# luigifcruz/radio-core

Hardware: AMD Instinct MI355X
Metric: IQ Msamples/s through Tuner+WBFM at 1024 channels (higher is better)
Workload: dtype f32

## Files before the change

### include/rcfm_tools.h

```cpp
#ifndef RCFM_TOOLS_H
#define RCFM_TOOLS_H

#include "rcfm.h"

#ifdef __cplusplus
extern "C" {
#endif

typedef struct rcfm_arena_s* rcfm_arena_t;

int rcfm_arena_create(size_t block_bytes, rcfm_arena_t* out);
int rcfm_arena_adopt(void* base, size_t bytes, rcfm_arena_t* out);
int rcfm_arena_bind(rcfm_arena_t arena);
int rcfm_arena_stats(rcfm_arena_t arena, size_t* reserved_bytes, size_t* used_bytes, size_t* live_pieces);
int rcfm_arena_destroy(rcfm_arena_t arena);


enum { RCFM_TUNER_OPT_NARROW_TILES = 1,
       RCFM_TUNER_OPT_ALIGNED_PLAN = 2 };
int rcfm_tuner_set_option(rcfm_tuner_t t, int option, int value);

enum { RCFM_OPT_LDS_CHAIN = 1, RCFM_OPT_FUSED_TILES = 2, RCFM_OPT_PHASE_LINK = 3, RCFM_OPT_PILOT_CHAIN = 6, RCFM_OPT_DECIM_TILE = 7,
       RCFM_OPT_LDS_DEEMPH = 8, RCFM_OPT_PILOT_BLOCKED = 9 };
int rcfm_demod_get_option(rcfm_demod_t d, int option, int* value);


typedef struct rcfm_fft_pass {
    int32_t L, nstages, radix[8];
    int64_t n_o1, n_o2, n_inner;
    int64_t in_o1, in_o2, in_i, in_l;
    int64_t out_o1, out_o2, out_i, out_k;
    int64_t tw_o1, tw_o2, tw_i;
    int32_t has_twiddle, load_along_l;
    int64_t in_t, out_t;
    int32_t flat_outer;
    int32_t reserved_;
} rcfm_fft_pass;
typedef struct rcfm_fft_plan {
// ... 23 lines not shown
```

### radio-core_amd/csrc/api_internal.h

```cpp
#pragma once

#include <algorithm>
#include <atomic>
#include <cstdlib>
#include <map>
#include <memory>
#include <mutex>
#include <string>
#include <vector>

#include "common.h"
#include "fft_engine.h"
#include "fft_plan.h"
#include "fused_passes.h"
#include "kernels.h"
#include "lds_chain.h"

#define TILE_CALL(narrow_tiles, fn, ...) ((narrow_tiles) ? ::rcfm::narrow::fn(__VA_ARGS__) : ::rcfm::fn(__VA_ARGS__))

namespace rcfm {

constexpr double kPi = 3.14159265358979323846;


// ... 1 lines not shown
    int64_t n = 0, m = 0;
    int nmin = 0, nyq = 0, nneg = 0;
    int nyq_mode = NYQ_NONE;
    float w_merge = 0.f;
    float nyq_factor = 1.f;
    float scale = 1.f;
    DeviceBuffer wpos, wneg;
    DeviceBuffer wr;

    void build(int64_t n_, int64_t m_, double a0, bool complex_input);
};

std::vector<double> firwin_bandpass(int numtaps, double lo, double hi);
std::vector<float> zero_phase_kernel(const float* b, int nb);
void deemphasis_design(int64_t fs, double tau, float* taps51, float* zi50);

struct PlanCache {
    std::map<int, std::unique_ptr<FftPlan>> by_batch;
    FftPlan& get(FftKind kind, size_t n, int batch, bool in_place, size_t& work_need) {
        auto it = by_batch.find(batch);
        if (it == by_batch.end())
            it = by_batch.emplace(batch, std::make_unique<FftPlan>(kind, n, (size_t)batch, in_place)).first;
        work_need = std::max(work_need, it->second->work_bytes());
        return *it->second;
    }
};

enum Stage : int {
    ST_TUNER_FFT = 0,
    ST_TUNER_GATHER,
// ... 174 lines not shown
```

### radio-core_amd/csrc/demod.hip

```cpp

#include <cmath>
#include <cstring>

#include "api_internal.h"

using namespace rcfm;

struct rcfm_demod_s {
    Arena* arena = arena_enter_handle();
    ~rcfm_demod_s() {
        drop_graphs();
        if (cap_stream) (void)hipStreamDestroy(cap_stream);
        arena_leave_handle(arena);
    }
    int kind = 0, C = 0, B = 0, A = 0, ch = 1, chunk = 1;
    double tau = 75e-6;
    float taps_h[51];
    float zi_h[50];
    float pilot_h[41];
    float pilot_g_h[41];
    DeviceBuffer taps, pilot_g;
    struct StateBuf : DeviceBuffer {
        hipEvent_t ev = nullptr;
        bool armed = false, recorded = false;
// ... 16 lines not shown
    float* state_ptr() const { return state_buf->as<float>() + state_off; }
    float* state_at(int first) const { return state_ptr() + (size_t)first * ch * 50; }
    float side_tap = 0.23f;
    ResampleGeom geom;
    PlanCache r2c_B, c2c_inv_B, c2c_fwd_B, c2c_inv_A, c2r_A;
    std::unique_ptr<FftEngine> eng_B, eng_A;
    std::unique_ptr<FftEngine> eng_Ad;
    std::unique_ptr<FftEngine> eng_Bi;
    DeviceBuffer buf_Ti;
    bool opt_lds_chain = true;
    bool opt_pilot_chain = true;
    bool opt_decim_tile = true;
    bool opt_pilot_blocked = true;
    bool opt_phase_link = true;
    bool opt_lds_deemph = true;
    int opt_narrow = kNarrowDefault;
    bool opt_graph = false;
    struct GraphSlot {
        const void* iq;
        void* audio;
        const float* state;
        int first;
        hipGraphExec_t exec;
        uint64_t used;
    };
    std::vector<GraphSlot> graphs;
    GraphSlot last_call{nullptr, nullptr, nullptr, -1, nullptr, 0};
    hipStream_t cap_stream = nullptr;
    uint64_t graph_tick = 0;
    void drop_graphs() {
// ... 92 lines not shown
    int audio_pitch() const {
        if (!eng_Ad || kind != RCFM_WBFM || !deemph_fused()) return 0;
        const int64_t n1 = eng_Ad->row_length();
        return (n1 % 16 == 0 || (n1 * 2) % 4 != 0) ? 0 : (int)((n1 + 15) / 16 * 16);
    }

    bool deemph_geometric() const {
        if (!(taps_h[0] == 0.f && taps_h[1] > 0.f)) return false;
        for (int i = 1; i < 50; ++i)
            if (std::fabs((double)taps_h[i + 1] * taps_h[1] - (double)taps_h[i] * taps_h[2]) >
                4e-7 * (double)taps_h[i] * taps_h[1] + 1e-36)
                return false;
        return true;
    }

    DeviceBuffer taps_sfx;
    const float* taps_sfx_dev() {
        if (taps_sfx.bytes() == 0) {
            float h[102];
            for (int i = 0; i < 51; ++i) h[i] = taps_h[i];
            double acc = 0.0;
            for (int i = 50; i >= 0; --i) {
                h[51 + i] = (float)acc;
                acc += (double)taps_h[i];
            }
            taps_sfx.upload(h, sizeof(h));
        }
        return taps_sfx.as<float>();
    }

// ... 100 lines not shown
            }
            paired = true;
        } else {
            {
                StageTimer tm(ST_FFT_REAL_B, s);
                TILE_CALL(nw, fused_real_pair_fft, *eng_B, p, U2, T, cnt, packed ? kKeepLowerHalf : -1, s);
            }
            if (eng_Bi && opt_pilot_chain) {
                StageTimer tm(ST_IFFT_B, s);
                paired = !packed ? TILE_CALL(nw, fused_hilbert_pair_ifft_mix_fft, *eng_Bi, *eng_B, U2, m, buf_Ti.as<float2>(), T, cnt, s)
                                 : TILE_CALL(nw, fused_hilbert_packed_ifft_mix_fft, *eng_Bi, *eng_B, U2, p, m,
                                             buf_Ti.as<float2>(), T, cnt, s);
            }
        }
        if (paired && eng_Ad && opt_decim_tile && TILE_CALL(nw, fused_fft_decim_ifft_applies, *eng_B, *eng_Ad, cnt)) {
            const int pitch = audio_pitch();
            {
                StageTimer tm(ST_FFT_B, s);
                TILE_CALL(nw, fused_fft_decim_ifft, *eng_B, *eng_Ad, T, V, TA, cnt, geom.wr.as<float>(), geom.scale,
                          buf_dc.as<float2>(), s, pitch);
            }
            run_deemph(reinterpret_cast<float*>(V), audio, first, cnt, s, false, pitch ? (int)eng_Ad->row_length() : 0, pitch);
            return;
        }
        if (paired) {
            StageTimer tm(ST_FFT_B, s);
            TILE_CALL(nw, fused_fft_last_pruned, *eng_B, T, Z, cnt, std::min(A, B) / 2, s);
        } else {
            {
                StageTimer tm(ST_IFFT_B, s);
// ... 291 lines not shown
    });
}

int rcfm_demod_set_option(rcfm_demod_t d, int option, int value) {
    return guarded([&] {
        RC_REQUIRE(d, RCFM_ERR_ARG, "NULL handle");
        d->drop_graphs();
        switch (option) {
            case RCFM_OPT_GRAPH: d->opt_graph = value != 0; break;
            case RCFM_OPT_LDS_CHAIN: d->opt_lds_chain = value != 0; break;
            case RCFM_OPT_FUSED_TILES: d->opt_pilot_chain = d->opt_decim_tile = value != 0; break;
            case RCFM_OPT_PILOT_CHAIN: d->opt_pilot_chain = value != 0; break;
            case RCFM_OPT_DECIM_TILE: d->opt_decim_tile = value != 0; break;
            case RCFM_OPT_PILOT_BLOCKED: d->opt_pilot_blocked = value != 0; break;
            case RCFM_OPT_LDS_DEEMPH: d->opt_lds_deemph = value != 0; break;
            case RCFM_OPT_PHASE_LINK: d->opt_phase_link = value != 0; break;
            case RCFM_OPT_NARROW_TILES:
                RC_REQUIRE(value >= 0 && value <= 2, RCFM_ERR_ARG, "narrow tiles: 0 never, 1 automatic, 2 always");
                d->opt_narrow = value;
                break;
            case RCFM_OPT_STATE_FENCE: {
                auto& b = *d->state_buf;
                if (value != 0 && b.ev == nullptr) RC_HIP(hipEventCreateWithFlags(&b.ev, hipEventDisableTiming));
                b.armed = value != 0;
                if (!b.armed) b.recorded = false;
                break;
            }
            default: RC_REQUIRE(false, RCFM_ERR_ARG, "unknown demodulator option");
        }
    });
}

int rcfm_demod_get_option(rcfm_demod_t d, int option, int* value) {
    return guarded([&] {
        RC_REQUIRE(d && value, RCFM_ERR_ARG, "NULL handle or output");
        switch (option) {
            case RCFM_OPT_LDS_CHAIN: *value = d->opt_lds_chain; break;
            case RCFM_OPT_FUSED_TILES: *value = d->opt_pilot_chain && d->opt_decim_tile; break;
            case RCFM_OPT_PILOT_CHAIN: *value = d->opt_pilot_chain; break;
            case RCFM_OPT_DECIM_TILE: *value = d->opt_decim_tile; break;
            case RCFM_OPT_PILOT_BLOCKED:
                *value = d->opt_pilot_blocked && d->opt_pilot_chain && d->pilot_blocked().valid() &&
                         fused_pilot_chain_applies(*d->eng_B, *d->eng_Bi, 2);
                break;
            case RCFM_OPT_LDS_DEEMPH: *value = d->opt_lds_deemph; break;
            case RCFM_OPT_PHASE_LINK: *value = d->opt_phase_link; break;
            case RCFM_OPT_NARROW_TILES: *value = d->opt_narrow; break;
            case RCFM_OPT_STATE_FENCE: *value = d->state_buf->armed; break;
            case RCFM_OPT_GRAPH: *value = d->opt_graph ? 1 + (int)d->graphs.size() : 0; break;
            default: RC_REQUIRE(false, RCFM_ERR_ARG, "unknown demodulator option");
        }
    });
}

int rcfm_demod_get_taps(rcfm_demod_t d, float* deemph51_host, float* pilot41_host) {
    return guarded([&] {
        RC_REQUIRE(d, RCFM_ERR_ARG, "NULL handle");
        if (deemph51_host) std::memcpy(deemph51_host, d->taps_h, sizeof(d->taps_h));
        if (pilot41_host) std::memcpy(pilot41_host, d->pilot_h, sizeof(d->pilot_h));
    });
// ... 50 lines not shown
```

### radio-core_amd/csrc/design.hip

```cpp

#include <cmath>

#include "api_internal.h"

namespace rcfm {

namespace {
double shifted_window(double a0, int64_t n, int64_t k) {
    if (n == 1) return 1.0;
    int64_t i = (k - n / 2) % n;
    if (i < 0) i += n;
    return a0 - (1.0 - a0) * std::cos(2.0 * kPi * (double)i / (double)n);
}
}

void ResampleGeom::build(int64_t n_, int64_t m_, double a0, bool complex_input) {
    n = n_;
    m = m_;
    nmin = (int)std::min(n, m);
    nyq = nmin / 2 + 1;
    scale = (float)(1.0 / (double)n);
    const bool even = (nmin % 2) == 0;
    if (complex_input) {
        nneg = nmin > 2 ? nmin - nyq : 0;
// ... 52 lines not shown
void deemphasis_design(int64_t fs, double tau, float* taps51, float* zi50) {
    const double x = std::exp(-1.0 / ((double)fs * tau));
    double st = 0.0, u = 1.0;
    for (int i = 0; i < 51; ++i) {
        taps51[i] = (float)((1.0 - x) * st);
        st = x * st + u;
        u = 0.0;
    }
    float acc = 0.f;
    for (int k = 49; k >= 0; --k) {
        acc += taps51[k + 1];
        zi50[k] = acc;
    }
}

}
```

### radio-core_amd/csrc/fft_decim_rt.h

```cpp
#pragma once

#include "fft_kernel.h"

namespace rcfm {
RCFM_NS_OPEN

struct WinAudioDecim {
    const float* wr;
    float2* dc;
    float scale;
    int A, n1;
    int split_count;
    __device__ __forceinline__ float weight(const fftk::LineId&, int l, int k0) const {
        const int kappa = l * n1 + k0;
        int kk = kappa <= A / 2 ? kappa : A - kappa;
        kk = kk < 0 ? 0 : kk;
        return wr[kk] * scale;
    }
    __device__ __forceinline__ void dc_bin(const fftk::LineId& id, float2 v) const {
        if (dc == nullptr) return;
        if (split_count > 0) {
            dc[2 * id.batch] = make_float2(v.x, 0.f);
            if (2 * id.batch + 1 < split_count) dc[2 * id.batch + 1] = make_float2(v.y, 0.f);
        } else {
            dc[id.batch] = v;
        }
    }
};

namespace fftk {

template <int R, int T>
__device__ __forceinline__ void stage_rt(float2* tile, const float2* tw, int L2, int mt, int tid) {
    const int m = mt / R, step = L2 / mt, nb = (L2 / R) * W;
    for (int e = tid; e < nb; e += T) {
        const int w = e & (W - 1), b = e >> kLogW;
        const int g = b / m, kp = b - g * m;
        const int base = g * mt + kp;
        float2 v[R];
#pragma unroll
        for (int q = 0; q < R; ++q) v[q] = tile[lds_slot<true>(base + q * m, w)];
        dft_p<R>(v);
        const int ts = kp * step;
#pragma unroll
        for (int q = 1; q < R; ++q) v[dft_slot<R>(q)] = cmul(v[dft_slot<R>(q)], tw[q * ts]);
#pragma unroll
        for (int q = 0; q < R; ++q) tile[lds_slot<true>(base + q * m, w)] = v[dft_slot<R>(q)];
    }
}

constexpr bool decim_rt_radix_ok(int r) {
    return r == 2 || r == 3 || r == 4 || r == 5 || r == 6 || r == 8 || r == 10 || r == 12 || r == 16;
}

template <int L, int R0, int R1, int R2, int R3, int T>
__global__ __launch_bounds__(T, (T * 16 / W >= 512 ? 4 : 1)) void k_fft_tile2_decim_rt(FftPassDev d1, FftPassDev d2,
                                                                              LoadPlainT<false> load, WinAudioDecim win,
                                                                              StorePlainT<false> store) {
    constexpr int S = (R0 > 1) + (R1 > 1) + (R2 > 1) + (R3 > 1);
    static_assert(S >= 2 && R0 * R1 * R2 * R3 == L, "bad radix list");
    constexpr int RL = (S == 2) ? R1 : (S == 3) ? R2 : R3;
    constexpr int RG = T / W;
    constexpr int nld = (L * W + T - 1) / T;
    constexpr int rowsL = L / RL, nitL = (rowsL + RG - 1) / RG;
    __shared__ __attribute__((aligned(16))) float2 tile[L * kRowsPitch];
    __shared__ __attribute__((aligned(16))) float2 tw[L];
    const FftPass& p1 = d1.p;
    const FftPass& p2 = d2.p;
    const int L2 = p2.L;
    const int tid = threadIdx.x;
    const int w = tid & (W - 1), rg = tid >> kLogW;

// ... 79 lines not shown
                else if (k == L2 / 2) l = L2;
                if (l >= 0) tile[lds_slot<true>(l, w)] = xr[it * RL + dft_slot<RL>(q)];
            }
        }
    }
    for (int e = tid; e < L2; e += T) tw[e] = d2.stage_tw[e];
    lds_barrier();

    for (int e = tid; e < L2 * W; e += T) {
        const int l = e >> kLogW, wl = e & (W - 1);
        float2 x = tile[lds_slot<true>(l, wl)];
        if (l == L2 / 2 && i0 + wl == 0) {
            const float2 y = tile[lds_slot<true>(L2, wl)];
            x = make_float2(x.x + y.x, x.y + y.y);
        }
        const float wg = win.weight(id, l, i0 + (wl < wvalid ? wl : 0));
        x = make_float2(x.x * wg, x.y * wg);
        if (l == 0 && i0 + wl == 0) {
            id.i = 0;
            win.dc_bin(id, x);
        }
        tile[lds_slot<true>(l, wl)] = make_float2(x.y, x.x);
    }
    lds_barrier();

    int mt = L2;
    for (int s = 0; s < p2.nstages; ++s) {
        const int r = p2.radix[s];
        switch (r) {
            case 2: stage_rt<2, T>(tile, tw, L2, mt, tid); break;
            case 3: stage_rt<3, T>(tile, tw, L2, mt, tid); break;
            case 4: stage_rt<4, T>(tile, tw, L2, mt, tid); break;
// ... 45 lines not shown
#define RCFM_CASE(LEN, A, B, C, D) have = have || d1.p.L == LEN;
    RCFM_FFT_DECIM_RT_LENGTHS(RCFM_CASE)
#undef RCFM_CASE
    const int L2 = d2.p.L;
    if (!have || (L2 & 1) || L2 < 16 || L2 >= d1.p.L) return false;
    for (int s = 0; s < d2.p.nstages; ++s)
        if (!decim_rt_radix_ok(d2.p.radix[s])) return false;
    return d1.p.load_along_l && !d2.p.load_along_l && d1.p.n_inner == d2.p.n_inner &&
           d1.p.n_o1 * d1.p.n_o2 == 1 && d2.p.n_o1 * d2.p.n_o2 == 1 && d1.p.out_k == d2.p.in_l && d2.p.in_i == 1 &&
           d2.p.out_i == 1 && d2.p.has_twiddle && batch <= 65535;
}

}

bool launch_fft_tile2_decim_rt(const FftPassDev& d1, const FftPassDev& d2, int batch, const float2* tmp_f,
                               const WinAudioDecim& win, float2* tmp_a, hipStream_t s);

RCFM_NS_CLOSE
}
```

### radio-core_amd/csrc/fft_kernel.h

```cpp
#pragma once

#include <hip/hip_runtime.h>

#include <cstdio>
#include <cstdlib>
#include <type_traits>

#include "fft_engine.h"
#include "tile_ns.h"

namespace rcfm {
RCFM_NS_OPEN
namespace fftk {

constexpr int W = RCFM_TILE_W;
constexpr int kLogW = W == 16 ? 4 : W == 8 ? 3 : 2;
static_assert((1 << kLogW) == W, "tile width: 4, 8 or 16 lines");
constexpr int kThreads = 256 * W / 16;

__device__ __forceinline__ float2 cmul(float2 a, float2 b) {
    typedef float v2f __attribute__((ext_vector_type(2)));
    v2f A, B, D;
    A.x = a.x; A.y = a.y; B.x = b.x; B.y = b.y;
    asm("v_pk_mul_f32 %0, %1, %2 op_sel:[0,0] op_sel_hi:[0,1]" : "=v"(D) : "v"(A), "v"(B));
// ... 1126 lines not shown
            const int q2 = r1 / w2, q3 = r1 - q2 * w2;
            return q1 + R0 * (q2 + R1 * q3);
        }
    };

    float2 v[nld];
#pragma unroll
    for (int it = 0; it < nld; ++it) {
        int e = tid + T * it;
        if ((L * W) % T != 0) e = e < L * W ? e : 0;
        const int wl = e / L, l = e - wl * L;
        const int wcl = wl < wvalid ? wl : 0;
        id.i = i0 + wcl;
        v[it] = load.fetch(id, l, in_base, (unsigned)wcl * in_i + (unsigned)l);
    }
    float wgt[nwin];
#pragma unroll
    for (int it = 0; it < nwin; ++it) {
        int e = tid + T * it;
        if ((L2 * W) % T != 0) e = e < L2 * W ? e : 0;
        const int wl = e & (W - 1);
        wgt[it] = win.weight(id, e >> kLogW, i0 + (wl < wvalid ? wl : 0));
    }
    for (int e = tid; e < L; e += T) tw[e] = d1.stage_tw[e];
#pragma unroll
    for (int it = 0; it < nld; ++it) {
        const int e = tid + T * it;
        const int wl = e / L, l = e - wl * L;
        id.i = i0 + wl;
        const float2 x = load.post(id, l, v[it]);
        if ((L * W) % T == 0 || e < L * W) tile[lds_slot<true>(l, wl)] = x;
// ... 39 lines not shown
        }
    }
    for (int e = tid; e < L2; e += T) tw[e] = d2.stage_tw[e];
    lds_barrier();

#pragma unroll
    for (int it = 0; it < nwin; ++it) {
        const int e = tid + T * it;
        if ((L2 * W) % T == 0 || e < L2 * W) {
            const int l = e >> kLogW, wl = e & (W - 1);
            float2 x = tile[lds_slot<true>(l, wl)];
            if (l == L2 / 2 && i0 + wl == 0) {
                const float2 y = tile[lds_slot<true>(L2, wl)];
                x = make_float2(x.x + y.x, x.y + y.y);
            }
            x = make_float2(x.x * wgt[it], x.y * wgt[it]);
            if (l == 0 && i0 + wl == 0) {
                id.i = 0;
                win.dc_bin(id, x);
            }
            tile[lds_slot<true>(l, wl)] = make_float2(x.y, x.x);
        }
    }
    lds_barrier();

    stage_lds<L2, Q0, L2, true, RG>(tile, tw, w, rg);
    lds_barrier();
    constexpr int rows2 = L2 / Q1;
    static_assert(rows2 <= RG, "short transform: one sweep");
    id.i = i0 + w;
    const unsigned f = (unsigned)((int64_t)(i0 + w) * p2.tw_i);
// ... 274 lines not shown
```

### radio-core_amd/csrc/fused_decim.hip

```cpp
#include "fft_decim_rt.h"

namespace rcfm {
RCFM_NS_OPEN

bool launch_fft_tile2_decim_rt(const FftPassDev& d1, const FftPassDev& d2, int batch, const float2* tmp_f,
                               const WinAudioDecim& win, float2* tmp_a, hipStream_t s) {
    using namespace fftk;
    if (!fft_tile2_decim_rt_applies(d1, d2, batch)) return false;
    const dim3 grid((unsigned)((d1.p.n_inner + W - 1) / W), 1, (unsigned)batch);
    LoadPlainT<false> ld{tmp_f};
    StorePlainT<false> st{tmp_a, 1.0f};
    switch (d1.p.L) {
#define RCFM_CASE(LEN, A, B, C, D)                                                                               \
    case LEN:                                                                                                    \
        hipLaunchKernelGGL((k_fft_tile2_decim_rt<LEN, A, B, C, D, tile_threads(LEN)>), grid,                     \
                           dim3(tile_threads(LEN)), 0, s, d1, d2, ld, win, st);                                  \
        break;
        RCFM_FFT_DECIM_RT_LENGTHS(RCFM_CASE)
#undef RCFM_CASE
        default: return false;
    }
    RC_HIP(hipGetLastError());
    return true;
}
// ... 4 lines not shown
```

### radio-core_amd/csrc/fused_passes.hip

```cpp
#include "fused_passes.h"
#include "device_math.h"

#include "fft_kernel.h"
#include "fft_decim_rt.h"
#include "kernels.h"

namespace rcfm {
RCFM_NS_OPEN

using fftk::LineId;
using fftk::kAnyPass;
using fftk::kRowsOnly;
using fftk::kStridedOnly;

namespace {


struct LoadTunerGatherFast {
    const float2* X;
    const int32_t* base;
    float two_pi_over_n, delta;
    float c0, c1, c2, c3;
    int B, nyq;
    int merge;
// ... 640 lines not shown
        RC_REQUIRE(fftk::launch_fft_tile2_pair(d1, d2, count, ld, mid, st, s), RCFM_ERR_RUNTIME,
                   "two-transform pair kernel refused a pair it should accept");
    }
}

void fused_fft_last_pruned(const FftEngine& e, const float2* tmp, float2* out, int count, int keep, hipStream_t s) {
    if (count <= 0) return;
    const int64_t n = e.desc().n;
    const int np = e.npass();
    fftk::LoadPlainT<false> ldl{tmp};
    StorePruned stl{out, (int)n, keep};
    fftk::launch_fft_pass<kRowsOnly>(e.pass_dev(np - 1, e.tmp_stride(), n), count, ldl, stl, s);
}

static bool decim_rt(const FftPassDev& d1, const FftPassDev& d2, int batch, const float2* tmp_f, const WinAudioDecim& win,
                     float2* tmp_a, hipStream_t s) {
    return launch_fft_tile2_decim_rt(d1, d2, batch, tmp_f, win, tmp_a, s);
}

bool fused_fft_decim_ifft_applies(const FftEngine& ef, const FftEngine& ea, int count) {
    if (ef.npass() != 2 || ea.npass() != 2) return false;
    const int64_t B = ef.desc().n, A = ea.desc().n;
    if (A >= B || (A & 1) || ea.desc().pass[1].L != ef.desc().pass[0].L) return false;
    const FftPassDev d1 = ef.pass_dev(1, ef.tmp_stride(), B), d2 = ea.pass_dev(0, A, ea.tmp_stride());
    return fftk::fft_tile2_decim_applies(d1, d2, count) || fftk::fft_tile2_decim_rt_applies(d1, d2, count);
}

void fused_fft_decim_ifft(const FftEngine& ef, const FftEngine& ea, const float2* tmp_f, float2* out, float2* tmp_a,
                          int count, const float* wr, float scale, float2* dc, hipStream_t s, int out_pitch) {
    if (count <= 0) return;
    const int64_t B = ef.desc().n, A = ea.desc().n;
    fftk::LoadPlainT<false> ld{tmp_f};
    WinAudioDecim win{wr, dc, scale, (int)A, ef.desc().pass[0].L, 0};
    fftk::StorePlainT<false> st{tmp_a, 1.0f};
    {
        const FftPassDev d1 = ef.pass_dev(1, ef.tmp_stride(), B), d2 = ea.pass_dev(0, A, ea.tmp_stride());
        RC_REQUIRE(fftk::launch_fft_tile2_decim(d1, d2, count, ld, win, st, s) || decim_rt(d1, d2, count, tmp_f, win, tmp_a, s),
                   RCFM_ERR_RUNTIME, "decimating two-transform kernel refused a pair it should accept");
    }
    fftk::LoadPlainT<false> ldl{tmp_a};
    fftk::StorePlainT<true> stl{out, 1.0f};
    FftPassDev last = ea.pass_dev(1, ea.tmp_stride(), A);
    if (out_pitch > 0) {
        RC_REQUIRE(out_pitch >= last.p.out_k && last.p.n_o1 * last.p.n_o2 == 1, RCFM_ERR_RUNTIME, "bad audio row pitch");
        last.out_batch = (A / last.p.out_k) * (int64_t)out_pitch;
        last.p.out_k = out_pitch;
    }
    fftk::launch_fft_pass<kRowsOnly>(last, count, ldl, stl, s);
}

struct StoreRealImagSplit {
    float* y;
    int n, count;
    __device__ __forceinline__ void operator()(const LineId& id, int, int64_t base, unsigned off, float2 v) const {
// ... 86 lines not shown
```

### radio-core_amd/csrc/fused_passes_decl.h

```cpp

namespace rcfm {
RCFM_DECL_NS_OPEN


void fused_tuner_ifft(const FftEngine& e, const TunerGather& g, float2* out, float2* tmp, int count,
                      hipStream_t s, float* theta = nullptr, int theta_pitch = 0);


void fused_real_fft(const FftEngine& e, const float* x, float2* U, float2* tmp, int count, int keep,
                    hipStream_t s);

void fused_hilbert_ifft(const FftEngine& e, const float2* U, float2* z, float2* tmp, int count, hipStream_t s);

void fused_real_pair_fft(const FftEngine& e, const float* x, float2* U2, float2* tmp, int count, int keep,
                         hipStream_t s, bool from_phase = false, PhaseRows rows = PhaseRows{});
void fused_hilbert_pair_ifft_mix(const FftEngine& e, const float2* U2, const float* m, float2* u, float2* tmp,
                                 int count, hipStream_t s);

bool fused_hilbert_pair_ifft_mix_fft(const FftEngine& ei, const FftEngine& ef, const float2* U2, const float* m,
                                     float2* tmp_i, float2* tmp_f, int count, hipStream_t s);
bool fused_hilbert_packed_applies(const FftEngine& ei, const FftEngine& ef, int count);
bool fused_hilbert_packed_ifft_mix_fft(const FftEngine& ei, const FftEngine& ef, const float2* U2, const float* p,
                                       const float* m, float2* tmp_i, float2* tmp_f, int count, hipStream_t s);
bool fused_pilot_chain_applies(const FftEngine& ef, const FftEngine& ei, int count);
bool fused_pilot_chain_geometry(const FftEngine& ef, int64_t* rows, int64_t* row_length);
void fused_pilot_chain_fft_first(const FftEngine& ef, const float* p, float2* tmp_f, int count, hipStream_t s,
                                 int64_t blk_stride = 0, int blk16 = 0);
void fused_pilot_chain_mask_mix(const FftEngine& ef, const FftEngine& ei, const float* p, const float* m,
                                float2* tmp_f, float2* tmp_i, int count, hipStream_t s, int64_t blk_stride = 0,
                                int blk16 = 0);

void fused_fft_last_pruned(const FftEngine& ef, const float2* tmp_f, float2* out, int count, int keep,
                           hipStream_t s);

bool fused_fft_decim_ifft_applies(const FftEngine& ef, const FftEngine& ea, int count);
void fused_fft_decim_ifft(const FftEngine& ef, const FftEngine& ea, const float2* tmp_f, float2* out, float2* tmp_a,
                          int count, const float* wr, float scale, float2* dc, hipStream_t s, int out_pitch = 0);

void fused_real_pair_fft_first(const FftEngine& e, const float* x, float2* tmp, int count, bool from_phase,
                               hipStream_t s, PhaseRows rows = PhaseRows{});
void fused_fft_decim_ifft_pairs(const FftEngine& ef, const FftEngine& ea, const float2* tmp_f, float* y,
                                float2* tmp_a, int count, const float* wr, float scale, float2* dc, hipStream_t s);

void fused_stereo_unpack_ifft(const FftEngine& e, const float2* U, int64_t B, float2* out, float2* tmp, int count,
                              const float* wr, int nyq, int nmin, float nyq_factor, float scale, float2* dc,
                              hipStream_t s);

void fused_fft_pruned(const FftEngine& e, const float2* in, float2* out, float2* tmp, int count, int keep,
                      hipStream_t s);

void fused_ifft_real_out(const FftEngine& e, const float2* Y, float* y, float2* tmp, int count, float scale,
                         hipStream_t s);

// ... 4 lines not shown
```

### radio-core_amd/csrc/kernels.h

```cpp
#pragma once

#include "common.h"

namespace rcfm {

enum NyquistMode : int { NYQ_NONE = 0, NYQ_DOWN = 1, NYQ_UP = 2 };

void launch_spectrum_c2c(const float2* X, int64_t x_stride, int64_t n, const int64_t* roll, float2* Y,
                         int64_t m, int batch, const float* wpos, const float* wneg, float w_merge,
                         int nyq, int nneg, int nyq_mode, float scale, hipStream_t stream);

void launch_spectrum_r2c(const float2* X, int64_t n, float2* Y, int64_t m, int batch, const float* wr,
                         int nyq, int nmin, float nyq_factor, float scale, hipStream_t stream);

void launch_spectrum_real_full(const float2* X, int64_t n, float2* Y, int64_t m, int batch, const float* wr,
                               int nyq, int nmin, float nyq_factor, float scale, float2* dc, bool paired,
                               hipStream_t stream);

void launch_hilbert_mask(const float2* P, float2* Z, int64_t n, int batch, float scale,
                         hipStream_t stream);

void launch_stereo_unpack(const float2* U, int64_t B, float2* V, int64_t A, int batch, const float* wr,
                          int nyq, int nmin, float nyq_factor, float scale, float2* dc, hipStream_t stream);

// ... 18 lines not shown
void launch_pilot_stage_h40_phase(const float* theta, float* m_out, float* p_out, int64_t n, int batch,
                                  const float* g_host, float side_tap, hipStream_t stream, const PilotBlocked* blk = nullptr);

void launch_stereo_mix(const float2* z, const float* m, float2* u, size_t count, hipStream_t stream);

void launch_pll_phase(const float2* z, size_t count, double mult, int want_imag, float* out,
                      hipStream_t stream);

int fir_tiles(int64_t n);
void launch_fir(const float* x, float* y, int64_t n, int ch, int batch, const float* taps, int nb,
                const float* state, float* partial, hipStream_t stream);
int fir51_tiles(int64_t n, int ch);
void launch_fir51(const float* x, float* y, int64_t n, int ch, int batch, const float* taps_host,
                  const float* state, float* partial, const float2* dc, hipStream_t stream, int row_samples = 0,
                  int row_pitch_samples = 0);
void launch_fir_state(const float* x, int64_t n, int ch, int batch, const float* taps, int nb,
                      float* state, hipStream_t stream, int row_samples = 0,
                      int row_pitch_samples = 0);
void launch_dc_clip(float* y, int64_t n, int ch, int batch, const float* partial, int nparts,
                    hipStream_t stream);

}
```

### radio-core_amd/csrc/kernels.hip

```cpp

#include "kernels.h"

#include <cmath>
#include "device_math.h"

namespace rcfm {

namespace {

constexpr int kThreads = 256;
constexpr float kInvPi = 0.31830988618379067154f;

__device__ __forceinline__ float2 cscale(float2 a, float s) { return make_float2(a.x * s, a.y * s); }

inline dim3 grid2(int64_t items, int per_block, int batch) {
    return dim3((unsigned)((items + per_block - 1) / per_block), (unsigned)batch, 1);
}


__global__ __launch_bounds__(kThreads) void k_spectrum_c2c(
    const float2* __restrict__ X, int64_t x_stride, int64_t n, const int64_t* __restrict__ roll,
    float2* __restrict__ Y, int64_t m, const float* __restrict__ wpos, const float* __restrict__ wneg,
    float w_merge, int nyq, int nneg, int nyq_mode, float scale) {
    const int c = blockIdx.y;
// ... 682 lines not shown
    for (int s = threadIdx.x; s < nb - 1; s += blockDim.x) {
        z_old[s] = zc[s];
        xt[s] = (s < n) ? xc[lay.at((n - 1 - s) * ch + h)] : 0.f;
    }
    for (int s = threadIdx.x; s < nb; s += blockDim.x) tp[s] = taps[s];
    __syncthreads();
    for (int s = threadIdx.x; s < nb - 1; s += blockDim.x) {
        float acc = 0.f;
        const int cnt = (int)((nb - 1 - s) < n ? (nb - 1 - s) : n);
        for (int i = 0; i < cnt; ++i) acc = fmaf(tp[s + 1 + i], xt[i], acc);
        if (s + n < nb - 1) acc += z_old[s + n];
        zc[s] = acc;
    }
}

__global__ __launch_bounds__(kThreads) void k_dc_clip(float* __restrict__ y, int64_t total,
                                                      const float* __restrict__ partial, int nparts) {
    __shared__ float mean_s;
    const int c = blockIdx.y;
    if (threadIdx.x < 64) {
        double acc = 0.0;
        for (int i = threadIdx.x; i < nparts; i += 64) acc += (double)partial[(int64_t)c * nparts + i];
        for (int off = 32; off > 0; off >>= 1) acc += __shfl_down(acc, off, 64);
        if (threadIdx.x == 0) mean_s = (float)(acc / (double)total);
    }
    __syncthreads();
    const float mean = mean_s;
    const int64_t i = (int64_t)blockIdx.x * kThreads + threadIdx.x;
    if (i >= total) return;
    float v = y[(int64_t)c * total + i] - mean;
// ... 168 lines not shown
    if (ch == 2)
        hipLaunchKernelGGL(k_fir51<2>, grid, dim3(kThreads), 0, stream, x, y, n * 2, taps, state, partial, dc, lay);
    else
        hipLaunchKernelGGL(k_fir51<1>, grid, dim3(kThreads), 0, stream, x, y, n, taps, state, partial, dc, lay);
    RC_LAUNCH_CHECK();
}

void launch_fir_state(const float* x, int64_t n, int ch, int batch, const float* taps, int nb,
                      float* state, hipStream_t stream, int row_samples, int row_pitch_samples) {
    if (batch <= 0 || nb < 2) return;
    hipLaunchKernelGGL(k_fir_state, dim3((unsigned)(batch * ch)), dim3(128), sizeof(float) * (3 * nb), stream,
                       x, n, ch, taps, nb, state, row_layout(n, ch, row_samples, row_pitch_samples));
    RC_LAUNCH_CHECK();
}

void launch_dc_clip(float* y, int64_t n, int ch, int batch, const float* partial, int nparts,
                    hipStream_t stream) {
    if (batch <= 0) return;
    const int64_t total = n * ch;
    hipLaunchKernelGGL(k_dc_clip, grid2(total, kThreads, batch), dim3(kThreads), 0, stream, y, total, partial,
                       nparts);
    RC_LAUNCH_CHECK();
}

}
```

### radio-core_amd/radiocore/_internal/hip.py

```python

import ctypes
import os
import sys
import threading
import warnings

import numpy as np

_HERE = os.path.dirname(os.path.abspath(__file__))
LIB_PATH = os.environ.get("RCFM_LIB") or os.path.join(os.path.dirname(_HERE), "_lib", "librcfm.so")

RCFM_FM, RCFM_MFM, RCFM_WBFM = 0, 1, 2
RCFM_OPT_LDS_CHAIN, RCFM_OPT_FUSED_TILES, RCFM_OPT_PHASE_LINK, RCFM_OPT_NARROW_TILES, RCFM_OPT_STATE_FENCE = 1, 2, 3, 4, 5
RCFM_OPT_PILOT_CHAIN, RCFM_OPT_DECIM_TILE, RCFM_OPT_LDS_DEEMPH, RCFM_OPT_PILOT_BLOCKED, RCFM_OPT_GRAPH = 6, 7, 8, 9, 10
RCFM_TUNER_OPT_NARROW_TILES, RCFM_TUNER_OPT_ALIGNED_PLAN = 1, 2

_ERR_SIZE, _ERR_INDEX, _ERR_RUNTIME, _ERR_ARG, _ERR_STATE = -1, -2, -3, -4, -5

_vp = ctypes.c_void_p
_i = ctypes.c_int
_i64 = ctypes.c_int64
_sz = ctypes.c_size_t
_dbl = ctypes.c_double
_fp = ctypes.POINTER(ctypes.c_float)

SIGNATURES = {
    "rcfm_version": [],
    "rcfm_device_count": [ctypes.POINTER(_i)],
    "rcfm_malloc": [ctypes.POINTER(_vp), _sz],
# ... 278 lines not shown
```

Before: 34490.

## Apply de-emphasis in frequency domain during decimating FFT and fuse DC-clip into IFFT store

Adds a spectral de-emphasis path for stereo WBFM. The 51-tap de-emphasis response is multiplied into the decimation window inside the fused FFT/decimate kernel. A small tail kernel evaluates the last samples by direct DFT to fix up the block boundary and state and to compute the mean. The final IFFT pass then stores the audio with the correction, DC removal and clipping folded in. This drops the separate time-domain FIR51, state and DC-clip passes, at the cost of a complex window multiply, a per-channel tail DFT kernel, and a circular-convolution approximation that relies on the geometric decay of the taps.

```diff
diff --git a/include/rcfm_tools.h b/include/rcfm_tools.h
--- a/include/rcfm_tools.h
+++ b/include/rcfm_tools.h
@@ -21,7 +21,7 @@
 int rcfm_tuner_set_option(rcfm_tuner_t t, int option, int value);
 
 enum { RCFM_OPT_LDS_CHAIN = 1, RCFM_OPT_FUSED_TILES = 2, RCFM_OPT_PHASE_LINK = 3, RCFM_OPT_PILOT_CHAIN = 6, RCFM_OPT_DECIM_TILE = 7,
-       RCFM_OPT_LDS_DEEMPH = 8, RCFM_OPT_PILOT_BLOCKED = 9 };
+       RCFM_OPT_LDS_DEEMPH = 8, RCFM_OPT_PILOT_BLOCKED = 9, RCFM_OPT_SPECTRAL_DEEMPH = 11 };
 int rcfm_demod_get_option(rcfm_demod_t d, int option, int* value);
 
 
diff --git a/radio-core_amd/csrc/api_internal.h b/radio-core_amd/csrc/api_internal.h
--- a/radio-core_amd/csrc/api_internal.h
+++ b/radio-core_amd/csrc/api_internal.h
@@ -39,6 +39,7 @@
 std::vector<double> firwin_bandpass(int numtaps, double lo, double hi);
 std::vector<float> zero_phase_kernel(const float* b, int nb);
 void deemphasis_design(int64_t fs, double tau, float* taps51, float* zi50);
+std::vector<float2> deemphasis_spectrum(const float* taps51, int64_t A);
 
 struct PlanCache {
     std::map<int, std::unique_ptr<FftPlan>> by_batch;
diff --git a/radio-core_amd/csrc/demod.hip b/radio-core_amd/csrc/demod.hip
--- a/radio-core_amd/csrc/demod.hip
+++ b/radio-core_amd/csrc/demod.hip
@@ -54,6 +54,7 @@
     bool opt_pilot_blocked = true;
     bool opt_phase_link = true;
     bool opt_lds_deemph = true;
+    bool opt_spectral_deemph = true;
     int opt_narrow = kNarrowDefault;
     bool opt_graph = false;
     struct GraphSlot {
@@ -176,6 +177,21 @@
         return true;
     }
 
+    DeviceBuffer deemph_spec, buf_corr, buf_mean;
+    bool spectral_deemph(bool nw) const {
+        return opt_spectral_deemph && kind == RCFM_WBFM && ch == 2 && eng_Ad && eng_Ad->row_length() % 16 == 0 &&
+               deemph_geometric() &&
+               deemph_tail_steps(taps_h, A) > 0 && ((int64_t)A * ch) % 4 == 0 &&
+               TILE_CALL(nw, fused_ifft_rows_audio_applies, *eng_Ad);
+    }
+    const float2* deemph_spec_dev() {
+        if (deemph_spec.bytes() == 0) {
+            const auto d = deemphasis_spectrum(taps_h, A);
+            deemph_spec.upload(d.data(), d.size() * sizeof(float2));
+        }
+        return deemph_spec.as<float2>();
+    }
+
     DeviceBuffer taps_sfx;
     const float* taps_sfx_dev() {
         if (taps_sfx.bytes() == 0) {
@@ -306,6 +322,26 @@
             }
         }
         if (paired && eng_Ad && opt_decim_tile && TILE_CALL(nw, fused_fft_decim_ifft_applies, *eng_B, *eng_Ad, cnt)) {
+            if (spectral_deemph(nw)) {
+                {
+                    StageTimer tm(ST_FFT_B, s);
+                    TILE_CALL(nw, fused_fft_decim_ifft_first, *eng_B, *eng_Ad, T, TA, cnt, geom.wr.as<float>(), geom.scale,
+                              buf_dc.as<float2>(), deemph_spec_dev(), s);
+                }
+                buf_corr.reserve((size_t)chunk * 50 * sizeof(float2));
+                buf_mean.reserve((size_t)chunk * sizeof(float));
+                {
+                    StateFence fence(*this, s);
+                    StageTimer tm(ST_DEEMPH_STATE, s);
+                    const FftPassDev last = eng_Ad->pass_dev(1, eng_Ad->tmp_stride(), A);
+                    launch_deemph_tail(TA, last.in_batch, last.p.in_i, last.p.in_l, (int)last.p.n_inner, last.p.L, cnt, taps_h,
+                                       state_at(first), buf_dc.as<float2>(), buf_corr.as<float2>(), buf_mean.as<float>(), s);
+                }
+                StageTimer tm(ST_DEEMPH, s);
+                TILE_CALL(nw, fused_ifft_rows_audio, *eng_Ad, TA, reinterpret_cast<float2*>(audio), cnt, buf_corr.as<float2>(),
+                          buf_mean.as<float>(), s);
+                return;
+            }
             const int pitch = audio_pitch();
             {
                 StageTimer tm(ST_FFT_B, s);
@@ -627,6 +663,7 @@
             case RCFM_OPT_DECIM_TILE: d->opt_decim_tile = value != 0; break;
             case RCFM_OPT_PILOT_BLOCKED: d->opt_pilot_blocked = value != 0; break;
             case RCFM_OPT_LDS_DEEMPH: d->opt_lds_deemph = value != 0; break;
+            case RCFM_OPT_SPECTRAL_DEEMPH: d->opt_spectral_deemph = value != 0; break;
             case RCFM_OPT_PHASE_LINK: d->opt_phase_link = value != 0; break;
             case RCFM_OPT_NARROW_TILES:
                 RC_REQUIRE(value >= 0 && value <= 2, RCFM_ERR_ARG, "narrow tiles: 0 never, 1 automatic, 2 always");
@@ -657,6 +694,7 @@
                          fused_pilot_chain_applies(*d->eng_B, *d->eng_Bi, 2);
                 break;
             case RCFM_OPT_LDS_DEEMPH: *value = d->opt_lds_deemph; break;
+            case RCFM_OPT_SPECTRAL_DEEMPH: *value = d->opt_spectral_deemph; break;
             case RCFM_OPT_PHASE_LINK: *value = d->opt_phase_link; break;
             case RCFM_OPT_NARROW_TILES: *value = d->opt_narrow; break;
             case RCFM_OPT_STATE_FENCE: *value = d->state_buf->armed; break;
diff --git a/radio-core_amd/csrc/design.hip b/radio-core_amd/csrc/design.hip
--- a/radio-core_amd/csrc/design.hip
+++ b/radio-core_amd/csrc/design.hip
@@ -90,4 +90,18 @@
     }
 }
 
+std::vector<float2> deemphasis_spectrum(const float* taps51, int64_t A) {
+    std::vector<float2> d((size_t)(A / 2 + 1));
+    for (int64_t k = 0; k <= A / 2; ++k) {
+        double re = 0.0, im = 0.0;
+        for (int j = 0; j < 51; ++j) {
+            const double ph = 2.0 * kPi * (double)((k * j) % A) / (double)A;
+            re += (double)taps51[j] * std::cos(ph);
+            im -= (double)taps51[j] * std::sin(ph);
+        }
+        d[(size_t)k] = make_float2((float)re, (float)im);
+    }
+    return d;
 }
+
+}
diff --git a/radio-core_amd/csrc/fft_decim_rt.h b/radio-core_amd/csrc/fft_decim_rt.h
--- a/radio-core_amd/csrc/fft_decim_rt.h
+++ b/radio-core_amd/csrc/fft_decim_rt.h
@@ -17,6 +17,7 @@
         kk = kk < 0 ? 0 : kk;
         return wr[kk] * scale;
     }
+    __device__ __forceinline__ float2 apply(float2 x, float wg) const { return make_float2(x.x * wg, x.y * wg); }
     __device__ __forceinline__ void dc_bin(const fftk::LineId& id, float2 v) const {
         if (dc == nullptr) return;
         if (split_count > 0) {
@@ -25,6 +26,23 @@
         } else {
             dc[id.batch] = v;
         }
+    }
+};
+
+struct WinAudioDecimDeemph : WinAudioDecim {
+    const float2* deemph;
+    __device__ __forceinline__ float2 weight(const fftk::LineId& id, int l, int k0) const {
+        const float g = WinAudioDecim::weight(id, l, k0);
+        if (deemph == nullptr) return make_float2(g, 0.f);
+        const int kappa = l * n1 + k0;
+        int kk = kappa <= A / 2 ? kappa : A - kappa;
+        kk = kk < 0 ? 0 : kk;
+        const float2 d = deemph[kk];
+        return make_float2(g * d.x, kappa <= A / 2 ? g * d.y : -g * d.y);
+    }
+    __device__ __forceinline__ float2 apply(float2 x, float2 wg) const {
+        if (deemph == nullptr) return make_float2(x.x * wg.x, x.y * wg.x);
+        return make_float2(x.x * wg.x - x.y * wg.y, x.x * wg.y + x.y * wg.x);
     }
 };
 
@@ -55,7 +73,7 @@
 
 template <int L, int R0, int R1, int R2, int R3, int T>
 __global__ __launch_bounds__(T, (T * 16 / W >= 512 ? 4 : 1)) void k_fft_tile2_decim_rt(FftPassDev d1, FftPassDev d2,
-                                                                              LoadPlainT<false> load, WinAudioDecim win,
+                                                                              LoadPlainT<false> load, WinAudioDecimDeemph win,
                                                                               StorePlainT<false> store) {
     constexpr int S = (R0 > 1) + (R1 > 1) + (R2 > 1) + (R3 > 1);
     static_assert(S >= 2 && R0 * R1 * R2 * R3 == L, "bad radix list");
@@ -165,8 +183,8 @@
             const float2 y = tile[lds_slot<true>(L2, wl)];
             x = make_float2(x.x + y.x, x.y + y.y);
         }
-        const float wg = win.weight(id, l, i0 + (wl < wvalid ? wl : 0));
-        x = make_float2(x.x * wg, x.y * wg);
+        const float2 wg = win.weight(id, l, i0 + (wl < wvalid ? wl : 0));
+        x = win.apply(x, wg);
         if (l == 0 && i0 + wl == 0) {
             id.i = 0;
             win.dc_bin(id, x);
@@ -242,7 +260,7 @@
 }
 
 bool launch_fft_tile2_decim_rt(const FftPassDev& d1, const FftPassDev& d2, int batch, const float2* tmp_f,
-                               const WinAudioDecim& win, float2* tmp_a, hipStream_t s);
+                               const WinAudioDecimDeemph& win, float2* tmp_a, hipStream_t s);
 
 RCFM_NS_CLOSE
 }
diff --git a/radio-core_amd/csrc/fft_kernel.h b/radio-core_amd/csrc/fft_kernel.h
--- a/radio-core_amd/csrc/fft_kernel.h
+++ b/radio-core_amd/csrc/fft_kernel.h
@@ -1164,7 +1164,7 @@
         id.i = i0 + wcl;
         v[it] = load.fetch(id, l, in_base, (unsigned)wcl * in_i + (unsigned)l);
     }
-    float wgt[nwin];
+    decltype(win.weight(id, 0, 0)) wgt[nwin];
 #pragma unroll
     for (int it = 0; it < nwin; ++it) {
         int e = tid + T * it;
@@ -1234,7 +1234,7 @@
                 const float2 y = tile[lds_slot<true>(L2, wl)];
                 x = make_float2(x.x + y.x, x.y + y.y);
             }
-            x = make_float2(x.x * wgt[it], x.y * wgt[it]);
+            x = win.apply(x, wgt[it]);
             if (l == 0 && i0 + wl == 0) {
                 id.i = 0;
                 win.dc_bin(id, x);
diff --git a/radio-core_amd/csrc/fused_decim.hip b/radio-core_amd/csrc/fused_decim.hip
--- a/radio-core_amd/csrc/fused_decim.hip
+++ b/radio-core_amd/csrc/fused_decim.hip
@@ -4,7 +4,7 @@
 RCFM_NS_OPEN
 
 bool launch_fft_tile2_decim_rt(const FftPassDev& d1, const FftPassDev& d2, int batch, const float2* tmp_f,
-                               const WinAudioDecim& win, float2* tmp_a, hipStream_t s) {
+                               const WinAudioDecimDeemph& win, float2* tmp_a, hipStream_t s) {
     using namespace fftk;
     if (!fft_tile2_decim_rt_applies(d1, d2, batch)) return false;
     const dim3 grid((unsigned)((d1.p.n_inner + W - 1) / W), 1, (unsigned)batch);
diff --git a/radio-core_amd/csrc/fused_passes.hip b/radio-core_amd/csrc/fused_passes.hip
--- a/radio-core_amd/csrc/fused_passes.hip
+++ b/radio-core_amd/csrc/fused_passes.hip
@@ -678,8 +678,11 @@
 }
 
 static bool decim_rt(const FftPassDev& d1, const FftPassDev& d2, int batch, const float2* tmp_f, const WinAudioDecim& win,
-                     float2* tmp_a, hipStream_t s) {
-    return launch_fft_tile2_decim_rt(d1, d2, batch, tmp_f, win, tmp_a, s);
+                     float2* tmp_a, hipStream_t s, const float2* deemph = nullptr) {
+    WinAudioDecimDeemph wd;
+    static_cast<WinAudioDecim&>(wd) = win;
+    wd.deemph = deemph;
+    return launch_fft_tile2_decim_rt(d1, d2, batch, tmp_f, wd, tmp_a, s);
 }
 
 bool fused_fft_decim_ifft_applies(const FftEngine& ef, const FftEngine& ea, int count) {
@@ -690,18 +693,78 @@
     return fftk::fft_tile2_decim_applies(d1, d2, count) || fftk::fft_tile2_decim_rt_applies(d1, d2, count);
 }
 
-void fused_fft_decim_ifft(const FftEngine& ef, const FftEngine& ea, const float2* tmp_f, float2* out, float2* tmp_a,
-                          int count, const float* wr, float scale, float2* dc, hipStream_t s, int out_pitch) {
+void fused_fft_decim_ifft_first(const FftEngine& ef, const FftEngine& ea, const float2* tmp_f, float2* tmp_a, int count,
+                                const float* wr, float scale, float2* dc, const float2* deemph, hipStream_t s) {
     if (count <= 0) return;
     const int64_t B = ef.desc().n, A = ea.desc().n;
     fftk::LoadPlainT<false> ld{tmp_f};
     WinAudioDecim win{wr, dc, scale, (int)A, ef.desc().pass[0].L, 0};
     fftk::StorePlainT<false> st{tmp_a, 1.0f};
-    {
-        const FftPassDev d1 = ef.pass_dev(1, ef.tmp_stride(), B), d2 = ea.pass_dev(0, A, ea.tmp_stride());
-        RC_REQUIRE(fftk::launch_fft_tile2_decim(d1, d2, count, ld, win, st, s) || decim_rt(d1, d2, count, tmp_f, win, tmp_a, s),
-                   RCFM_ERR_RUNTIME, "decimating two-transform kernel refused a pair it should accept");
-    }
+    const FftPassDev d1 = ef.pass_dev(1, ef.tmp_stride(), B), d2 = ea.pass_dev(0, A, ea.tmp_stride());
+    bool ok;
+    if (deemph != nullptr) {
+        WinAudioDecimDeemph wd;
+        static_cast<WinAudioDecim&>(wd) = win;
+        wd.deemph = deemph;
+        ok = fftk::launch_fft_tile2_decim(d1, d2, count, ld, wd, st, s);
+    } else {
+        ok = fftk::launch_fft_tile2_decim(d1, d2, count, ld, win, st, s);
+    }
+    RC_REQUIRE(ok || decim_rt(d1, d2, count, tmp_f, win, tmp_a, s, deemph), RCFM_ERR_RUNTIME,
+               "decimating two-transform kernel refused a pair it should accept");
+}
+
+struct StoreAudioFinish {
+    float2* out;
+    const float2* corr;
+    const float* mean;
+    int A;
+    __device__ __forceinline__ void operator()(const LineId& id, int, int64_t base, unsigned off, float2 v) const {
+        const int64_t g = base + off;
+        const int64_t t = g - (int64_t)id.batch * A;
+        float2 y = make_float2(v.y, v.x);
+        if (t < 50) {
+            const float2 c = corr[(int64_t)id.batch * 50 + t];
+            y = make_float2(y.x + c.x, y.y + c.y);
+        }
+        const float mu = mean[id.batch];
+        y.x -= mu;
+        y.y -= mu;
+        y.x = (y.x < -0.999f) ? -0.999f : ((y.x > 0.999f) ? 0.999f : y.x);
+        y.y = (y.y < -0.999f) ? -0.999f : ((y.y > 0.999f) ? 0.999f : y.y);
+        if constexpr (fftk::W == 16) {
+            const bool straddle =
+                ((reinterpret_cast<uintptr_t>(out + g) - ((uintptr_t)((int)id.i & (fftk::W - 1)) << 3)) & 127u) != 0;
+            if (straddle) {
+                asm volatile("global_store_dwordx2 %0, %1, off sc1" : : "v"(out + g), "v"(y) : "memory");
+                return;
+            }
+        }
+        fftk::stream_store(out + g, y);
+    }
+};
+
+bool fused_ifft_rows_audio_applies(const FftEngine& ea) {
+    if (ea.npass() != 2) return false;
+    const FftPass& p = ea.desc().pass[1];
+    return p.n_o1 * p.n_o2 == 1 && p.out_i == 1 && p.out_k == ea.desc().pass[0].L && !p.has_twiddle;
+}
+
+void fused_ifft_rows_audio(const FftEngine& ea, const float2* tmp_a, float2* audio, int count, const float2* corr,
+                           const float* mean, hipStream_t s) {
+    if (count <= 0) return;
+    const int64_t A = ea.desc().n;
+    RC_REQUIRE((fused_ifft_rows_audio_applies)(ea), RCFM_ERR_RUNTIME, "IFFT_A's last pass does not store natural order");
+    fftk::LoadPlainT<false> ldl{tmp_a};
+    StoreAudioFinish stl{audio, corr, mean, (int)A};
+    fftk::launch_fft_pass<kRowsOnly>(ea.pass_dev(1, ea.tmp_stride(), A), count, ldl, stl, s);
+}
+
+void fused_fft_decim_ifft(const FftEngine& ef, const FftEngine& ea, const float2* tmp_f, float2* out, float2* tmp_a,
+                          int count, const float* wr, float scale, float2* dc, hipStream_t s, int out_pitch) {
+    if (count <= 0) return;
+    const int64_t A = ea.desc().n;
+    (fused_fft_decim_ifft_first)(ef, ea, tmp_f, tmp_a, count, wr, scale, dc, nullptr, s);
     fftk::LoadPlainT<false> ldl{tmp_a};
     fftk::StorePlainT<true> stl{out, 1.0f};
     FftPassDev last = ea.pass_dev(1, ea.tmp_stride(), A);
diff --git a/radio-core_amd/csrc/fused_passes_decl.h b/radio-core_amd/csrc/fused_passes_decl.h
--- a/radio-core_amd/csrc/fused_passes_decl.h
+++ b/radio-core_amd/csrc/fused_passes_decl.h
@@ -37,6 +37,12 @@
 void fused_fft_decim_ifft(const FftEngine& ef, const FftEngine& ea, const float2* tmp_f, float2* out, float2* tmp_a,
                           int count, const float* wr, float scale, float2* dc, hipStream_t s, int out_pitch = 0);
 
+void fused_fft_decim_ifft_first(const FftEngine& ef, const FftEngine& ea, const float2* tmp_f, float2* tmp_a, int count,
+                                const float* wr, float scale, float2* dc, const float2* deemph, hipStream_t s);
+bool fused_ifft_rows_audio_applies(const FftEngine& ea);
+void fused_ifft_rows_audio(const FftEngine& ea, const float2* tmp_a, float2* audio, int count, const float2* corr,
+                           const float* mean, hipStream_t s);
+
 void fused_real_pair_fft_first(const FftEngine& e, const float* x, float2* tmp, int count, bool from_phase,
                                hipStream_t s, PhaseRows rows = PhaseRows{});
 void fused_fft_decim_ifft_pairs(const FftEngine& ef, const FftEngine& ea, const float2* tmp_f, float* y,
diff --git a/radio-core_amd/csrc/kernels.h b/radio-core_amd/csrc/kernels.h
--- a/radio-core_amd/csrc/kernels.h
+++ b/radio-core_amd/csrc/kernels.h
@@ -56,6 +56,10 @@
 void launch_fir51(const float* x, float* y, int64_t n, int ch, int batch, const float* taps_host,
                   const float* state, float* partial, const float2* dc, hipStream_t stream, int row_samples = 0,
                   int row_pitch_samples = 0);
+int deemph_tail_steps(const float* taps_host, int64_t A);
+void launch_deemph_tail(const float2* ta, int64_t in_batch, int64_t in_i, int64_t in_l, int rows, int len, int batch,
+                        const float* taps_host, float* state, const float2* dc, float2* corr, float* mean,
+                        hipStream_t stream);
 void launch_fir_state(const float* x, int64_t n, int ch, int batch, const float* taps, int nb,
                       float* state, hipStream_t stream, int row_samples = 0,
                       int row_pitch_samples = 0);
diff --git a/radio-core_amd/csrc/kernels.hip b/radio-core_amd/csrc/kernels.hip
--- a/radio-core_amd/csrc/kernels.hip
+++ b/radio-core_amd/csrc/kernels.hip
@@ -1,6 +1,7 @@
 
 #include "kernels.h"
 
+#include <algorithm>
 #include <cmath>
 #include "device_math.h"
 
@@ -720,6 +721,84 @@
     }
 }
 
+struct TailGeom {
+    int64_t in_batch, in_i, in_l;
+    int rows, len;
+    int steps;
+    float a, inv_c, a50;
+};
+
+constexpr int kTailThreads = 256;
+constexpr int kTailMaxSteps = 8;
+
+__global__ __launch_bounds__(kTailThreads) void k_deemph_tail(const float2* __restrict__ ta, TailGeom g,
+                                                              DeemphTaps taps, float* __restrict__ state,
+                                                              const float2* __restrict__ dc,
+                                                              float2* __restrict__ corr, float* __restrict__ mean) {
+    __shared__ float2 ys[50 * kTailMaxSteps + 1];
+    __shared__ float2 xs[50];
+    const int c = blockIdx.x;
+    const int tid = threadIdx.x, lane = tid & 63, wave = tid >> 6;
+    const int A = g.rows * g.len;
+    const int ns = 50 * g.steps + 1;
+    const float2* tc = ta + (int64_t)c * g.in_batch;
+    for (int i = wave; i < ns; i += kTailThreads / 64) {
+        const int t = (i == ns - 1) ? 0 : A - 50 * g.steps + i;
+        const int k1 = t % g.rows, k2 = t / g.rows;
+        const float2* row = tc + (int64_t)k1 * g.in_i;
+        float2 acc = make_float2(0.f, 0.f);
+        for (int n2 = lane; n2 < g.len; n2 += 64) {
+            const float2 v = row[(int64_t)n2 * g.in_l];
+            const int m = (int)(((int64_t)n2 * k2) % g.len);
+            float sn, cs;
+            sincospif(2.f * (float)m / (float)g.len, &sn, &cs);
+            acc.x = fmaf(v.x, cs, fmaf(v.y, sn, acc.x));
+            acc.y = fmaf(v.y, cs, fmaf(-v.x, sn, acc.y));
+        }
+        for (int off = 32; off > 0; off >>= 1) {
+            acc.x += __shfl_down(acc.x, off, 64);
+            acc.y += __shfl_down(acc.y, off, 64);
+        }
+        if (lane == 0) ys[i] = make_float2(acc.y, acc.x);
+    }
+    __syncthreads();
+    if (tid < 50) {
+        float2 x = make_float2(0.f, 0.f);
+        float w = g.inv_c;
+        for (int m = 0; m < g.steps; ++m) {
+            const int i = 50 * (g.steps - 1 - m) + tid;
+            const float2 y1 = ys[i + 1], y0 = ys[i];
+            x.x = fmaf(w, fmaf(-g.a, y0.x, y1.x), x.x);
+            x.y = fmaf(w, fmaf(-g.a, y0.y, y1.y), x.y);
+            w *= g.a50;
+        }
+        xs[tid] = x;
+    }
+    __syncthreads();
+    float2 cr = make_float2(0.f, 0.f);
+    if (tid < 50) {
+        float2 zf = make_float2(0.f, 0.f);
+        for (int j = tid + 1; j <= 50; ++j) {
+            const float2 x = xs[50 + tid - j];
+            zf.x = fmaf(taps.b[j], x.x, zf.x);
+            zf.y = fmaf(taps.b[j], x.y, zf.y);
+        }
+        float* st = state + (int64_t)c * 100;
+        cr = make_float2(st[tid] - zf.x, st[50 + tid] - zf.y);
+        corr[(int64_t)c * 50 + tid] = cr;
+        st[tid] = zf.x;
+        st[50 + tid] = zf.y;
+    }
+    if (wave == 0) {
+        float sum = cr.x + cr.y;
+        for (int off = 32; off > 0; off >>= 1) sum += __shfl_down(sum, off, 64);
+        if (lane == 0) {
+            const float2 d = dc[c];
+            mean[c] = ((float)A * (d.x + d.y) + sum) / (float)(2 * A);
+        }
+    }
+}
+
 __global__ __launch_bounds__(kThreads) void k_dc_clip(float* __restrict__ y, int64_t total,
                                                       const float* __restrict__ partial, int nparts) {
     __shared__ float mean_s;
@@ -918,6 +997,30 @@
     RC_LAUNCH_CHECK();
 }
 
+int deemph_tail_steps(const float* taps_host, int64_t A) {
+    if (!(taps_host[0] == 0.f && taps_host[1] > 0.f && taps_host[2] > 0.f)) return 0;
+    const double a = (double)taps_host[2] / taps_host[1];
+    if (!(a > 0.0 && a < 1.0)) return 0;
+    const int steps = std::max(1, (int)std::ceil(std::log(1e-6) / (50.0 * std::log(a))));
+    return (steps <= kTailMaxSteps && A >= 50 * (int64_t)steps + 51) ? steps : 0;
+}
+
+void launch_deemph_tail(const float2* ta, int64_t in_batch, int64_t in_i, int64_t in_l, int rows, int len, int batch,
+                        const float* taps_host, float* state, const float2* dc, float2* corr, float* mean,
+                        hipStream_t stream) {
+    if (batch <= 0) return;
+    const int steps = deemph_tail_steps(taps_host, (int64_t)rows * len);
+    RC_REQUIRE(steps > 0, RCFM_ERR_RUNTIME, "de-emphasis tail: taps or length outside the spectral form");
+    DeemphTaps taps;
+    for (int i = 0; i < 51; ++i) taps.b[i] = taps_host[i];
+    const double a = (double)taps_host[2] / taps_host[1];
+    const TailGeom g{in_batch, in_i, in_l, rows, len, steps, (float)a, (float)(1.0 / taps_host[1]),
+                     (float)(a * taps_host[50] / taps_host[1])};
+    hipLaunchKernelGGL(k_deemph_tail, dim3((unsigned)batch), dim3(kTailThreads), 0, stream, ta, g, taps, state, dc,
+                       corr, mean);
+    RC_LAUNCH_CHECK();
+}
+
 void launch_dc_clip(float* y, int64_t n, int ch, int batch, const float* partial, int nparts,
                     hipStream_t stream) {
     if (batch <= 0) return;
diff --git a/radio-core_amd/radiocore/_internal/hip.py b/radio-core_amd/radiocore/_internal/hip.py
--- a/radio-core_amd/radiocore/_internal/hip.py
+++ b/radio-core_amd/radiocore/_internal/hip.py
@@ -13,6 +13,7 @@
 RCFM_FM, RCFM_MFM, RCFM_WBFM = 0, 1, 2
 RCFM_OPT_LDS_CHAIN, RCFM_OPT_FUSED_TILES, RCFM_OPT_PHASE_LINK, RCFM_OPT_NARROW_TILES, RCFM_OPT_STATE_FENCE = 1, 2, 3, 4, 5
 RCFM_OPT_PILOT_CHAIN, RCFM_OPT_DECIM_TILE, RCFM_OPT_LDS_DEEMPH, RCFM_OPT_PILOT_BLOCKED, RCFM_OPT_GRAPH = 6, 7, 8, 9, 10
+RCFM_OPT_SPECTRAL_DEEMPH = 11
 RCFM_TUNER_OPT_NARROW_TILES, RCFM_TUNER_OPT_ALIGNED_PLAN = 1, 2
 
 _ERR_SIZE, _ERR_INDEX, _ERR_RUNTIME, _ERR_ARG, _ERR_STATE = -1, -2, -3, -4, -5
```

Result: no change. 34530, median of 6 (+0.1%).
